# codeslake/RefVSR

Hardware: AMD Instinct MI355X
Metric: 4x SR frames/sec (270p->1080p, RefVSR_small_L1) (higher is better)
Workload: dtype f16

## Files before the change

### refvsr_amd/csrc/common.h

```cpp
#pragma once
#include <stdlib.h>
#include <hip/hip_runtime.h>
#include <hip/hip_fp16.h>
#include <stdint.h>
#include <stdio.h>
#include <string.h>

#include "../../include/refvsr_hip.h"

typedef _Float16 f16;
typedef f16 f16x2 __attribute__((ext_vector_type(2)));
typedef f16 f16x4 __attribute__((ext_vector_type(4)));
typedef f16 f16x8 __attribute__((ext_vector_type(8)));
typedef float f32x4 __attribute__((ext_vector_type(4)));
typedef float f32x16 __attribute__((ext_vector_type(16)));

void refvsr_set_error(const char* fmt, ...);

#define RV_CHECK(cond, ...)                        \
    do {                                           \
        if (!(cond)) {                             \
            refvsr_set_error(__VA_ARGS__);         \
            return 1;                              \
        }                                          \
    } while (0)

#define RV_HIP(call)                                                                  \
    do {                                                                              \
        hipError_t e_ = (call);                                                       \
        if (e_ != hipSuccess) {                                                       \
            refvsr_set_error("%s failed: %s (%s:%d)", #call, hipGetErrorString(e_), __FILE__, __LINE__); \
            return 2;                                                                 \
        }                                                                             \
    } while (0)

#define RV_LAUNCH_CHECK() RV_HIP(hipGetLastError())

static inline int rv_cdiv(int a, int b) { return (a + b - 1) / b; }

#define RV_MAX_DEVICES 16
static inline int rv_device() {
    int d = 0;
    if (hipGetDevice(&d) != hipSuccess || d < 0 || d >= RV_MAX_DEVICES) d = 0;
    return d;
}
static inline int rv_num_cus() {
    static int n_cu[RV_MAX_DEVICES] = {};
    const int d = rv_device();
    if (n_cu[d] == 0) {
        hipDeviceProp_t prop;
        if (hipGetDeviceProperties(&prop, d) == hipSuccess) n_cu[d] = prop.multiProcessorCount;
        if (n_cu[d] <= 0) n_cu[d] = 256;
    }
    return n_cu[d];
}

int rv_stream_cus(hipStream_t st);

__device__ __forceinline__ void rv_tile_range(const int n_tiles, const int g, int& t_begin, int& t_end) {
    const int b = (int)blockIdx.x;
    int rank = b;
    if (g >= 8) {
        const int xcd = b & 7;
        rank = b >> 3;
        for (int y = 0; y < xcd; ++y) rank += (g - y + 7) >> 3;
    }
    const unsigned un = (unsigned)n_tiles, ug = (unsigned)g;
    t_begin = (int)(((unsigned)rank * un) / ug);
    t_end = (int)(((unsigned)(rank + 1) * un) / ug);
}

__device__ __forceinline__ int rv_reflect(int i, int n) {
    i = i < 0 ? -i : i;
    return i >= n ? 2 * (n - 1) - i : i;
}

__device__ __forceinline__ float rv_lrelu(float v, float slope) { return v >= 0.f ? v : v * slope; }

__device__ __forceinline__ float rv_linspace_m1p1(int j, int n) {
    const float step = 2.0f / (float)(n - 1);
    return (j < n / 2) ? (-1.0f + step * (float)j) : (1.0f - step * (float)(n - 1 - j));
}

struct WarpCoord { int x0, y0; float w00, w01, w10, w11; bool v00, v01, v10, v11; };

__device__ __forceinline__ WarpCoord warp_coord_uv(const float u, const float v, int hf, int wf, int hin, int win, int y, int x);
__device__ __forceinline__ WarpCoord warp_coord(const float* flow, int hf, int wf, int hin, int win, int y, int x) {
    const size_t fp = (size_t)y * wf + x;
    return warp_coord_uv(flow[fp], flow[(size_t)hf * wf + fp], hf, wf, hin, win, y, x);
}
__device__ __forceinline__ WarpCoord warp_coord_uv(const float u, const float v, int hf, int wf, int hin, int win, int y, int x) {
    const float gx = rv_linspace_m1p1(x, wf) + u / (((float)win - 1.0f) / 2.0f);
    const float gy = rv_linspace_m1p1(y, hf) + v / (((float)hin - 1.0f) / 2.0f);
    const float xs = ((gx + 1.0f) * (float)win - 1.0f) / 2.0f;
    const float ys = ((gy + 1.0f) * (float)hin - 1.0f) / 2.0f;
    const float fx = floorf(xs), fy = floorf(ys);
    const float tx = xs - fx, ty = ys - fy;
    WarpCoord c;
    c.x0 = (int)fminf(fmaxf(fx, -2.0f), (float)win + 1.0f);
    c.y0 = (int)fminf(fmaxf(fy, -2.0f), (float)hin + 1.0f);
    const bool xin0 = c.x0 >= 0 && c.x0 < win, xin1 = c.x0 + 1 >= 0 && c.x0 + 1 < win;
    const bool yin0 = c.y0 >= 0 && c.y0 < hin, yin1 = c.y0 + 1 >= 0 && c.y0 + 1 < hin;
    c.v00 = xin0 && yin0; c.v01 = xin1 && yin0; c.v10 = xin0 && yin1; c.v11 = xin1 && yin1;
    c.w00 = (1.0f - ty) * (1.0f - tx); c.w01 = (1.0f - ty) * tx;
    c.w10 = ty * (1.0f - tx); c.w11 = ty * tx;
    return c;
}

__device__ __forceinline__ uint4 warp_group16(const unsigned char* x, int pixb, int hin, int win, const WarpCoord& c, int goff) {
    float acc[8] = {0, 0, 0, 0, 0, 0, 0, 0};
    auto tap = [&](bool valid, int yy, int xx, float wgt) {
        if (valid) {
            const f16x8 v = *reinterpret_cast<const f16x8*>(x + ((size_t)yy * win + xx) * pixb + goff);
#pragma unroll
            for (int k = 0; k < 8; ++k) acc[k] += wgt * (float)v[k];
        }
    };
    tap(c.v00, c.y0, c.x0, c.w00);
    tap(c.v01, c.y0, c.x0 + 1, c.w01);
    tap(c.v10, c.y0 + 1, c.x0, c.w10);
    tap(c.v11, c.y0 + 1, c.x0 + 1, c.w11);
    union { f16x8 h; uint4 u; } o;
#pragma unroll
    for (int k = 0; k < 8; ++k) o.h[k] = (f16)acc[k];
    return o.u;
}

__device__ __forceinline__ void rv_bilinear_ac_src(int o, int n_in, int n_out, int& i0, int& i1, float& l1) {
#pragma clang fp contract(off)
    const float sc = n_out > 1 ? (float)(n_in - 1) / (float)(n_out - 1) : 0.0f;
    const float x = (float)o * sc;
    i0 = min((int)x, n_in - 1);
    i1 = min(i0 + 1, n_in - 1);
    l1 = x - (float)i0;
}
__device__ __forceinline__ float rv_bilinear_ac2_at(const float* __restrict__ s, int h, int w, int oy, int ox) {
    int y0, y1, x0, x1;
    float ly, lx;
    rv_bilinear_ac_src(oy, h, 2 * h, y0, y1, ly);
    rv_bilinear_ac_src(ox, w, 2 * w, x0, x1, lx);
    const float wy0 = 1.0f - ly, wx0 = 1.0f - lx;
    const float r0 = fmaf(lx, s[(size_t)y0 * w + x1], fmaf(wx0, s[(size_t)y0 * w + x0], 0.0f));
    const float r1 = fmaf(lx, s[(size_t)y1 * w + x1], fmaf(wx0, s[(size_t)y1 * w + x0], 0.0f));
    return fmaf(ly, r1, fmaf(wy0, r0, 0.0f));
}

__device__ __forceinline__ void rv_cubic_taps(float t, float* wgt) {
    const float A = -0.75f;
    float x = t + 1.0f;
    wgt[0] = ((A * x - 5.0f * A) * x + 8.0f * A) * x - 4.0f * A;
    x = t;
    wgt[1] = ((A + 2.0f) * x - (A + 3.0f)) * x * x + 1.0f;
    x = 1.0f - t;
    wgt[2] = ((A + 2.0f) * x - (A + 3.0f)) * x * x + 1.0f;
    x = 2.0f - t;
    wgt[3] = ((A * x - 5.0f * A) * x + 8.0f * A) * x - 4.0f * A;
}
__device__ __forceinline__ void rv_cubic_src(int o, int n_in, float scale, int* idx, float* wgt) {
    const float x = ((float)o + 0.5f) * scale - 0.5f;
    const float fl = floorf(x);
    const int ix = (int)fl;
    rv_cubic_taps(x - fl, wgt);
#pragma unroll
    for (int k = 0; k < 4; ++k) idx[k] = min(max(ix - 1 + k, 0), n_in - 1);
}
__device__ __forceinline__ float rv_bicubic_at(const float* __restrict__ s, int h, int w, int oy, int ox, float sy, float sx) {
    int iy[4], ix[4];
    float wy[4], wx[4];
    rv_cubic_src(oy, h, sy, iy, wy);
    rv_cubic_src(ox, w, sx, ix, wx);
    float acc = 0.0f;
#pragma unroll
    for (int j = 0; j < 4; ++j) {
        float r = 0.0f;
        const float* row = s + (size_t)iy[j] * w;
#pragma unroll
        for (int i = 0; i < 4; ++i) r = fmaf(wx[i], row[ix[i]], r);
        acc = fmaf(wy[j], r, acc);
    }
    return acc;
}

__device__ __forceinline__ void rv_store_result(void* out, const size_t e, const float v, const int fmt) {
    if (fmt == REFVSR_RESULT_F32) reinterpret_cast<float*>(out)[e] = v;
    else if (fmt == REFVSR_RESULT_F16) reinterpret_cast<f16*>(out)[e] = (f16)v;
    else reinterpret_cast<unsigned char*>(out)[e] = (unsigned char)__float2int_rn(v * 255.0f);
}

__host__ __device__ inline int rv_keven(int ks, int ncg) {
    const int ce = (ncg + 1) >> 1, co = ncg >> 1;
    return ks * (((ks + 1) >> 1) * ce + (ks >> 1) * co);
}
__host__ __device__ inline int rv_ksteps(int ks, int ncg) { return (ks * ks * ncg + (rv_keven(ks, ncg) & 1) + 3) / 4; }
__host__ __device__ inline int rv_kslot(int ty, int tx, int cg, int ks, int ncg) {
    const int ce = (ncg + 1) >> 1, co = ncg >> 1;
    const int p = (tx + cg) & 1;
    const int c0 = p ? co : ce, c1 = p ? ce : co;
    const int row = ((ks + 1) >> 1) * c0 + (ks >> 1) * c1;
    const int rank = ty * row + ((tx + 1) >> 1) * c0 + (tx >> 1) * c1 + (cg >> 1);
    if (!p) return rank;
    const int E = rv_keven(ks, ncg);
    return E + (E & 1) + rank;
}
__host__ __device__ inline int rv_kpad_slot(int j, int ks, int ncg) {
    const int E = rv_keven(ks, ncg);
    return ((E & 1) && j == 0) ? E : ks * ks * ncg + j;
}
__device__ __forceinline__ int rv_pix16(int n) { return (n < 4 || n >= 12) ? ((n & 7) << 1) : (((n - 4) << 1) | 1); }
```

### refvsr_amd/csrc/conv_mfma.hip

```cpp
#include <type_traits>

#include "common.h"
#include <stdlib.h>

#define CONV_CH 8
#define CONV_RES_MAX 16
#define CONV_XPF 8
#define CONV_TW 32

struct ConvArgs {
    const unsigned char* src0; const unsigned char* src1;
    int c0, c1, ncg0, ncg, ps;
    int pixb0, pixb1;
    int h_in, w_in, h_out, w_out;
    int ks, stride, pad;
    int LH, LW;
    int G, S;
    float inv_ncg;
    const uint4* wpack; const float* bias;
    int cout;
    float act_slope, post_slope;
    const unsigned char* mul; int mul_c;
    const unsigned char* res; int res_c;
    int out_mode; void* out; int out_c;
// ... 455 lines not shown
            auto ld128 = [](const unsigned addr) {
                u32x4 v;
                asm volatile("ds_read_b128 %0, %1" : "=v"(v) : "v"(addr));
                return make_uint4(v[0], v[1], v[2], v[3]);
            };
            auto tie = [](uint4& r) {
                u32x4 t = {r.x, r.y, r.z, r.w};
                asm volatile("" : "+v"(t));
                r = make_uint4(t[0], t[1], t[2], t[3]);
            };
            auto wait_set = [&](uint4 (&a)[NA], uint4 (&b)[TILES]) {
                asm volatile("s_waitcnt lgkmcnt(%0)" :: "n"(NA + TILES) : "memory");
#pragma unroll
                for (int i = 0; i < NA; ++i) tie(a[i]);
#pragma unroll
                for (int t = 0; t < TILES; ++t) tie(b[t]);
            };
            static_assert(NA + TILES <= 15, "lgkmcnt range");
            auto compute_chunk = [&](const unsigned wslot, const int s0, const int ns) {
                unsigned toff[CONV_CH];
#pragma unroll
                for (int j = 0; j < CONV_CH; ++j)
                    asm volatile("ds_read_b32 %0, %1" : "=v"(toff[j]) : "v"(lds_tab + (unsigned)(((s0 + min(j, ns - 1)) * 4 + q) * 4)));
                asm volatile("s_waitcnt lgkmcnt(0)" ::: "memory");
#pragma unroll
                for (int j = 0; j < CONV_CH; ++j) asm volatile("" : "+v"(toff[j]));
                const unsigned wa = wslot + (unsigned)lane * 16;
                auto load_set = [&](auto jc, uint4 (&a)[NA], uint4 (&b)[TILES]) {
                    constexpr int j = decltype(jc)::value;
                    const unsigned wj = wa + (unsigned)min(j, ns - 1) * (NA * 1024);
#pragma unroll
                    for (int i = 0; i < NA; ++i) {
                        u32x4 v;
                        asm volatile("ds_read_b128 %0, %1 offset:%2" : "=v"(v) : "v"(wj), "n"(i * 1024));
                        a[i] = make_uint4(v[0], v[1], v[2], v[3]);
                    }
#pragma unroll
                    for (int t = 0; t < TILES; ++t) b[t] = ld128(pbaddr[t] + toff[j]);
                };
                uint4 a0[NA], b0[TILES], a1[NA], b1[TILES];
                load_set(std::integral_constant<int, 0>{}, a0, b0);
#define RV_RING_PAIR(J)                                                                     \
                load_set(std::integral_constant<int, (J) + 1>{}, a1, b1);                   \
                wait_set(a0, b0);                                                           \
                __builtin_amdgcn_sched_barrier(0);                                          \
                if ((J) < ns) mfma_step(a0, b0);                                            \
                load_set(std::integral_constant<int, (J) + 2>{}, a0, b0);                   \
                wait_set(a1, b1);                                                           \
                __builtin_amdgcn_sched_barrier(0);                                          \
                if ((J) + 1 < ns) mfma_step(a1, b1);
                RV_RING_PAIR(0) RV_RING_PAIR(2) RV_RING_PAIR(4)
#undef RV_RING_PAIR
                static_assert(CONV_CH == 8, "the ring loop is unrolled for 8 K-steps per chunk");
                load_set(std::integral_constant<int, 7>{}, a1, b1);
                wait_set(a0, b0);
                __builtin_amdgcn_sched_barrier(0);
                if (6 < ns) mfma_step(a0, b0);
                asm volatile("s_waitcnt lgkmcnt(0)" ::: "memory");
#pragma unroll
                for (int i = 0; i < NA; ++i) tie(a1[i]);
#pragma unroll
                for (int t = 0; t < TILES; ++t) tie(b1[t]);
                __builtin_amdgcn_sched_barrier(0);
                if (7 < ns) mfma_step(a1, b1);
            };
            const int n_chunks = (p.S + CONV_CH - 1) / CONV_CH;
            zero_acc();
            int slot_r = 0;
            for (int c = 0; c < n_chunks; ++c) {
                const int after = min(NS - 2, n_chunks - 1 - c);
                if (after <= 0) asm volatile("s_waitcnt vmcnt(0)" ::: "memory");
                else if (after == 1) asm volatile("s_waitcnt vmcnt(%0)" :: "n"(PPW) : "memory");
                else asm volatile("s_waitcnt vmcnt(%0)" :: "n"(2 * PPW) : "memory");
                asm volatile("s_waitcnt lgkmcnt(0)" ::: "memory");
                __builtin_amdgcn_s_barrier();
                asm volatile("" ::: "memory");
                if (c + NS - 1 < n_chunks) { issue(c + NS - 1, slot_w); slot_w = slot_w + 1 == NS ? 0 : slot_w + 1; }
                compute_chunk(lds_wl + (unsigned)slot_r * SLOT, c * CONV_CH, min(CONV_CH, p.S - c * CONV_CH));
                slot_r = slot_r + 1 == NS ? 0 : slot_r + 1;
            }
        } else {
            constexpr int WPT = (CONV_CH * MT * WFR * 64) / NT;
            const int n_chunks = (p.S + CONV_CH - 1) / CONV_CH;
            static_assert(WPT <= 12, "prefetch register set");
            uint4 w0, w1, w2, w3, w4, w5, w6, w7, w8, w9, w10, w11;
    #define RV_W_ALL(OP) OP(0) OP(1) OP(2) OP(3) OP(4) OP(5) OP(6) OP(7) OP(8) OP(9) OP(10) OP(11)
    #define RV_W_LOAD(k) if constexpr (WPT > k) w##k = g[min(tid + k * NT, n16n - 1)];
    #define RV_W_STORE(k) if constexpr (WPT > k) { if (tid + k * NT < n16n) d[tid + k * NT] = w##k; }
            {
                const int n16 = min(CONV_CH, p.S) * MT * WFR * 64;
                uint4* d = reinterpret_cast<uint4*>(wl);
                for (int i = tid; i < n16; i += NT) d[i] = wsrc[i];
            }
            zero_acc();
            __syncthreads();
            for (int c = 0; c < n_chunks; ++c) {
                const int s0 = c * CONV_CH;
                const int ns = min(CONV_CH, p.S - s0);
                const bool has_next = (c + 1 < n_chunks);
                const int sn = has_next ? s0 + CONV_CH : s0;
                const int n16n = min(CONV_CH, p.S - sn) * MT * WFR * 64;
                {
                    const uint4* g = wsrc + (size_t)sn * MT * WFR * 64;
                    RV_W_ALL(RV_W_LOAD)
                }
                compute_steps(wl, s0, ns);
                if (has_next) {
                    __syncthreads();
                    uint4* d = reinterpret_cast<uint4*>(wl);
                    RV_W_ALL(RV_W_STORE)
                    __syncthreads();
                }
            }
        }
        epilogue(ty0, tx0, tid);
    }
}

static int g_wg_cap = 0;
extern "C" int refvsr_set_conv_workgroup_cap(int cap) {
    g_wg_cap = cap > 0 ? cap : 0;
    return 0;
}

extern "C" int refvsr_kslot(int ty, int tx, int cg, int ksize, int ncg) { return rv_kslot(ty, tx, cg, ksize, ncg); }
extern "C" int refvsr_ksteps(int ksize, int ncg) { return rv_ksteps(ksize, ncg); }

template <int MT, int TILES, bool F32, bool GATHER, bool RESIDENT, int EPI = 0, int NW = 4, bool HI1 = false>
static int launch_conv(ConvArgs& a, int nz, size_t lds, hipStream_t st) {
    static bool attr_done[RV_MAX_DEVICES] = {};
    const int dev = rv_device();
    if (!attr_done[dev]) {
        RV_HIP(hipFuncSetAttribute(reinterpret_cast<const void*>(&conv_mfma_kernel<MT, TILES, F32, GATHER, RESIDENT, EPI, NW, HI1>),
                                   hipFuncAttributeMaxDynamicSharedMemorySize, 160 * 1024));
        attr_done[dev] = true;
    }
    int gx = a.n_xy;
    if (RESIDENT) {
        static size_t occ_lds[RV_MAX_DEVICES][4] = {};
        static int occ_val[RV_MAX_DEVICES][4] = {};
        static int slot[RV_MAX_DEVICES] = {};
        int occ = 0;
        for (int i = 0; i < 4; ++i)
            if (occ_lds[dev][i] == lds && occ_val[dev][i] > 0) occ = occ_val[dev][i];
        if (occ == 0) {
            RV_HIP(hipOccupancyMaxActiveBlocksPerMultiprocessor(&occ, conv_mfma_kernel<MT, TILES, F32, GATHER, RESIDENT, EPI, NW, HI1>, NW * 64, lds));
            if (occ < 1) occ = 1;
            occ_lds[dev][slot[dev] & 3] = lds; occ_val[dev][slot[dev] & 3] = occ; ++slot[dev];
        }
        int cap = (rv_stream_cus(st) * occ / (nz * (a.batch > 1 ? a.batch : 1))) & ~7;
        if (cap < 8) cap = 8;
        if (g_wg_cap > 0) cap = g_wg_cap;
        if (gx > cap) gx = cap;
    }
    a.grid = gx;
    hipLaunchKernelGGL((conv_mfma_kernel<MT, TILES, F32, GATHER, RESIDENT, EPI, NW, HI1>), dim3(gx, a.batch > 1 ? a.batch : 1, nz), dim3(NW * 64), lds, st, a);
    RV_LAUNCH_CHECK();
    return 0;
}

extern "C" int refvsr_conv_mfma(const RefvsrConv* d, void* stream) {
    RV_CHECK(d != nullptr, "conv: null descriptor");
    const bool f32 = d->f32 == 1;
    const bool hi1 = d->f32 == 2;
    RV_CHECK(d->f32 >= 0 && d->f32 <= 2, "conv: weight mode (f32) must be 0, 1 or 2");
    const int cgrp = f32 ? 4 : 8;
    const int esz = f32 ? 4 : 2;
    RV_CHECK(d->src0 && d->c0 > 0 && d->c0 % cgrp == 0, "conv: src0/c0 invalid (c0=%d)", d->c0);
    RV_CHECK((d->src1 == nullptr) == (d->c1 == 0) && d->c1 % cgrp == 0, "conv: src1/c1 invalid (c1=%d)", d->c1);
    RV_CHECK(d->ksize >= 1 && d->ksize <= 7 && d->stride >= 1 && d->pad >= 0, "conv: bad geometry");
    RV_CHECK(d->h_in > 0 && d->w_in > 0 && d->h_out > 0 && d->w_out > 0, "conv: bad sizes");
    RV_CHECK(d->wpack && d->bias && d->out, "conv: null weights/bias/out");
    RV_CHECK(d->mt_per_block >= 1 && d->mt_per_block <= 3, "conv: mt_per_block must be 1..3");
    RV_CHECK(d->cout >= 1, "conv: cout");
    if (d->out_mode != REFVSR_OUT_PLANAR32) {
        RV_CHECK(d->cout % 4 == 0 && d->out_c % 4 == 0, "conv: nhwc16 output needs cout %% 4 == 0");
        RV_CHECK(d->res_planar == nullptr, "conv: res_planar only with planar output");
    }
    if (d->out_mode == REFVSR_OUT_NHWC16_SHUFFLE2)
        RV_CHECK(d->cout % 16 == 0 && !d->mul && !d->res && !f32 && d->out_c >= d->cout / 4 && d->out_c - d->cout / 4 <= 4,
                 "conv: pixel-shuffle output constraints");
    RV_CHECK(refvsr_init() == 0, "init failed");

    ConvArgs a;
    memset(&a, 0, sizeof(a));
    a.src0 = (const unsigned char*)d->src0; a.src1 = (const unsigned char*)d->src1;
    a.c0 = d->c0; a.c1 = d->c1;
    a.pixb0 = d->c0 * esz; a.pixb1 = d->c1 * esz;
    a.ncg0 = d->c0 / cgrp; a.ncg = (d->c0 + d->c1) / cgrp;
    a.ps = a.ncg | 1;
    a.h_in = d->h_in; a.w_in = d->w_in; a.h_out = d->h_out; a.w_out = d->w_out;
    a.ks = d->ksize; a.stride = d->stride; a.pad = d->pad;
    a.G = d->ksize * d->ksize * a.ncg;
    a.S = rv_ksteps(d->ksize, a.ncg);
    RV_CHECK(a.S == d->ksteps, "conv: ksteps mismatch (descriptor %d, geometry %d)", d->ksteps, a.S);
    a.inv_ncg = 1.0f / (float)a.ncg;
    a.wpack = (const uint4*)d->wpack; a.bias = d->bias; a.cout = d->cout;
    a.act_slope = d->act_slope; a.post_slope = d->post_slope;
    a.mul = (const unsigned char*)d->mul; a.mul_c = d->mul_c;
    a.res = (const unsigned char*)d->res; a.res_c = d->res_c;
    a.out_mode = d->out_mode; a.out = d->out; a.out_c = d->out_c;
    a.res_planar = d->res_planar; a.add_const = d->add_const;
    a.clamp_lo = d->clamp_lo; a.clamp_hi = d->clamp_hi;
    RV_CHECK(d->batch >= 0 && d->batch <= 65535, "conv: batch out of range (%d)", d->batch);
    a.batch = d->batch > 1 ? d->batch : 1;
    if (a.batch > 1) {
        RV_CHECK(!d->mul && !d->res, "conv: batch > 1 takes no mul / res operands");
        RV_CHECK(d->bs_src0 % 16 == 0 && d->bs_src1 % 16 == 0 && d->bs_out % 8 == 0 && d->bs_res_planar % 4 == 0, "conv: batch strides must keep the maps aligned");
        RV_CHECK(d->bs_src0 > 0 && d->bs_out > 0 && (!d->src1 || d->bs_src1 > 0) && (!d->res_planar || d->bs_res_planar > 0), "conv: batch strides missing");
        a.bs_src0 = d->bs_src0; a.bs_src1 = d->bs_src1; a.bs_out = d->bs_out; a.bs_res_planar = d->bs_res_planar;
    }

    const int MT = d->mt_per_block;
    const int n_mt = (d->cout + 15) / 16;
    const int nz = (n_mt + MT - 1) / MT;
    a.tab_bytes = ((a.S * 4 * 4 + 15) / 16) * 16;
    const int wfr_kb = MT * ((f32 || hi1) ? 1 : 2) * 1024;
    static const bool no_resident = getenv("REFVSR_CONV_NO_PERSIST") != nullptr;
    const size_t LDS_MAX = 160 * 1024;

    int tiles = 4;
    size_t lds = 0;
    auto tile_bytes = [&](int tl) {
        a.LH = (tl * 2 - 1) * a.stride + a.ks;
        a.LW = (CONV_TW - 1) * a.stride + a.ks;
        return (size_t)a.LH * a.LW * a.ps * 16;
    };
    bool resident = false, one_wg = false;
    bool w16 = false;
    static const int res_max = getenv("REFVSR_CONV_RES_MAX") ? atoi(getenv("REFVSR_CONV_RES_MAX")) : CONV_RES_MAX;
    if (!no_resident && !hi1 && a.S <= res_max && a.S <= CONV_RES_MAX) {
        int best_wg = 0;
        static const int force_tiles = getenv("REFVSR_CONV_TILES") ? atoi(getenv("REFVSR_CONV_TILES")) : 0;
        for (int tl = 4; tl >= 2; tl -= 2) {
            if (force_tiles && tl != force_tiles) continue;
            const size_t tb = tile_bytes(tl);
            const size_t need = (size_t)a.tab_bytes + (size_t)a.S * wfr_kb + tb;
            const int chunks = a.LH * a.LW * a.ncg;
            const int wg = need <= LDS_MAX ? (int)(LDS_MAX / need) : 0;
            if (chunks > CONV_XPF * 256 || wg == 0) continue;
            if (a.LH > 31 || a.LW > 127 || a.ncg > 127) continue;
            if (best_wg == 0 || (best_wg < 2 && wg > best_wg)) { best_wg = wg; tiles = tl; lds = need; resident = true; }
        }
        if (resident) { a.wl_bytes = a.S * wfr_kb; tile_bytes(tiles); one_wg = best_wg == 1; }
        static const bool no_w16 = getenv("REFVSR_CONV_NO_W16") != nullptr;
        if (resident && one_wg && tiles == 4 && !f32 && !no_w16 && (MT == 2 || MT == 3)) {
            const size_t tb = tile_bytes(8);
            const size_t need = (size_t)a.tab_bytes + (size_t)a.S * wfr_kb + tb;
            const int chunks = a.LH * a.LW * a.ncg;
            if (need <= LDS_MAX && chunks <= 4096 && a.LH <= 31 && a.LW <= 127) { tiles = 8; lds = need; w16 = true; }
            else tile_bytes(tiles);
        }
    }
    if (!resident) {
        const size_t slot = (size_t)CONV_CH * wfr_kb;
        const int n_chunks = (a.S + CONV_CH - 1) / CONV_CH;
        auto ring_for = [&](int tl, size_t budget) {
            const size_t fixed = (size_t)a.tab_bytes + tile_bytes(tl);
            if (fixed + 2 * slot > budget) return 0;
            int ns = (int)((budget - fixed) / slot);
            if (ns > 4) ns = 4;
            if (ns > n_chunks + 1) ns = n_chunks + 1 > 2 ? n_chunks + 1 : 2;
            return ns;
        };
        static const int force_ring = getenv("REFVSR_CONV_RING") ? atoi(getenv("REFVSR_CONV_RING")) : 0;
        const bool big = (long long)d->h_out * d->w_out > 64 * 1024;
        int ns = 0;
        tiles = 4;
        if (big) ns = ring_for(4, LDS_MAX / 2);
        if (!ns && big) { tiles = 2; ns = ring_for(2, LDS_MAX / 2); }
        if (!ns) { tiles = 4; ns = ring_for(4, LDS_MAX); }
        if (!ns) { tiles = 2; ns = ring_for(2, LDS_MAX); }
        if (ns) {
            if (force_ring >= 2 && force_ring < ns) ns = force_ring;
            a.ring = ns;
            a.wl_bytes = (int)(ns * slot);
            lds = (size_t)a.tab_bytes + (size_t)a.wl_bytes + tile_bytes(tiles);
        } else {
            a.gather = 1;
            a.ring = 1;
            tiles = 4;
            a.LH = a.LW = 0;
            a.wl_bytes = (int)slot;
            lds = (size_t)a.tab_bytes + (size_t)a.wl_bytes;
            RV_CHECK(d->h_in < 60000 && d->w_in < 60000, "conv: frame too large for gather-mode coordinates");
        }
        one_wg = !a.gather && lds > LDS_MAX / 2;
    }
    static const bool no_nw8 = getenv("REFVSR_CONV_NO_NW8") != nullptr;
    const int n_tiles8 = rv_cdiv(d->w_out, CONV_TW) * rv_cdiv(d->h_out, 8);
    const bool nw8 = tiles == 4 && !f32 && !a.gather && !no_nw8 && (one_wg || n_tiles8 <= 2048);
    static const bool no_prefetch = getenv("REFVSR_CONV_NO_PREFETCH") != nullptr;
    a.prefetch = no_prefetch ? 0 : 1;
    a.tiles_x = rv_cdiv(d->w_out, CONV_TW);
    a.n_xy = a.tiles_x * rv_cdiv(d->h_out, tiles * 2);
    hipStream_t st = (hipStream_t)stream;
    if (a.gather) {
        RV_CHECK(!f32 && !hi1, "conv: gather mode is built for the fp16 hi+lo path only");
        if (MT == 1) return launch_conv<1, 4, false, true, false>(a, nz, lds, st);
        if (MT == 2) return launch_conv<2, 4, false, true, false>(a, nz, lds, st);
        return launch_conv<3, 4, false, true, false>(a, nz, lds, st);
    }
    if (hi1) {
        RV_CHECK(!a.gather && MT <= 2, "conv: single-fp16 weights are built for the streamed stride-1 convs (MT=%d)", MT);
        const bool nw8h = tiles == 4 && !no_nw8 && (one_wg || n_tiles8 <= 2048);
        if (nw8h) return MT == 1 ? launch_conv<1, 2, false, false, false, 0, 8, true>(a, nz, lds, st)
                                 : launch_conv<2, 2, false, false, false, 0, 8, true>(a, nz, lds, st);
        if (tiles == 4) return MT == 1 ? launch_conv<1, 4, false, false, false, 0, 4, true>(a, nz, lds, st)
                                       : launch_conv<2, 4, false, false, false, 0, 4, true>(a, nz, lds, st);
        return MT == 1 ? launch_conv<1, 2, false, false, false, 0, 4, true>(a, nz, lds, st)
                       : launch_conv<2, 2, false, false, false, 0, 4, true>(a, nz, lds, st);
    }
    static const bool no_lean = getenv("REFVSR_CONV_NO_LEAN_EPI") != nullptr;
    const bool lean = resident && !f32 && !no_lean && d->out_mode == REFVSR_OUT_NHWC16 && d->act_slope >= 0.f && d->act_slope <= 1.f &&
                      d->post_slope >= 0.f && d->post_slope <= 1.f &&
                      (long long)d->h_out * d->w_out * (long long)(d->out_c > d->mul_c ? (d->out_c > d->res_c ? d->out_c : d->res_c)
                                                                                       : (d->mul_c > d->res_c ? d->mul_c : d->res_c)) < (1ll << 31);
#define RV_CONV_CASE(M, T)                                                                                \
    if (MT == M && tiles == T) {                                                                          \
        if (f32) return resident ? launch_conv<M, T, true, false, true>(a, nz, lds, st)                   \
                                 : launch_conv<M, T, true, false, false>(a, nz, lds, st);                 \
        if (lean) return launch_conv<M, T, false, false, true, 1>(a, nz, lds, st);                        \
        return resident ? launch_conv<M, T, false, false, true>(a, nz, lds, st)                           \
                        : launch_conv<M, T, false, false, false>(a, nz, lds, st);                         \
    }
    if (w16) {
        if (MT == 3) return lean ? launch_conv<3, 2, false, false, true, 1, 16>(a, nz, lds, st) : launch_conv<3, 2, false, false, true, 0, 16>(a, nz, lds, st);
        return lean ? launch_conv<2, 2, false, false, true, 1, 16>(a, nz, lds, st) : launch_conv<2, 2, false, false, true, 0, 16>(a, nz, lds, st);
    }
    if (nw8) {
#define RV_CONV_CASE8(M)                                                                                  \
        if (MT == M) {                                                                                    \
            if (lean) return launch_conv<M, 2, false, false, true, 1, 8>(a, nz, lds, st);                 \
            return resident ? launch_conv<M, 2, false, false, true, 0, 8>(a, nz, lds, st)                 \
                            : launch_conv<M, 2, false, false, false, 0, 8>(a, nz, lds, st);               \
        }
        RV_CONV_CASE8(1) RV_CONV_CASE8(2) RV_CONV_CASE8(3)
#undef RV_CONV_CASE8
    }
    if (!no_nw8 && f32 && tiles == 2 && !a.gather && (MT == 1 || MT == 2)) {
        if (MT == 1) return resident ? launch_conv<1, 1, true, false, true, 0, 8>(a, nz, lds, st) : launch_conv<1, 1, true, false, false, 0, 8>(a, nz, lds, st);
        return resident ? launch_conv<2, 1, true, false, true, 0, 8>(a, nz, lds, st) : launch_conv<2, 1, true, false, false, 0, 8>(a, nz, lds, st);
    }
    RV_CONV_CASE(1, 2) RV_CONV_CASE(1, 4)
    RV_CONV_CASE(2, 2) RV_CONV_CASE(2, 4)
    RV_CONV_CASE(3, 2) RV_CONV_CASE(3, 4)
#undef RV_CONV_CASE
    refvsr_set_error("conv: no kernel for MT=%d tiles=%d", MT, tiles);
    return 1;
}
```

Before: 235.3.

## Add specialized 7x7 SPyNet conv kernel with pipelined weight streaming

Adds a dedicated MFMA kernel for the stride-1 7x7 SPyNet convolutions (32->64, 64->32, 32->16 channels) and routes the single-fp16-weight conv path to it when shapes match. The kernel stages an input tile in LDS and streams weight chunks into a multi-slot LDS ring via global_load_lds. It uses hand-scheduled ds_read and waitcnt double-buffering around the MFMAs. This targets the heavy 7x7 flow-network convolutions that the generic conv kernel handles less efficiently, at the cost of fixed shape-specific configurations and inline-asm fragility.

```diff
diff --git a/refvsr_amd/csrc/common.h b/refvsr_amd/csrc/common.h
--- a/refvsr_amd/csrc/common.h
+++ b/refvsr_amd/csrc/common.h
@@ -56,6 +56,8 @@
 }
 
 int rv_stream_cus(hipStream_t st);
+
+int rv_spynet7_conv(const RefvsrConv* d, hipStream_t st);
 
 __device__ __forceinline__ void rv_tile_range(const int n_tiles, const int g, int& t_begin, int& t_end) {
     const int b = (int)blockIdx.x;
diff --git a/refvsr_amd/csrc/conv_mfma.hip b/refvsr_amd/csrc/conv_mfma.hip
--- a/refvsr_amd/csrc/conv_mfma.hip
+++ b/refvsr_amd/csrc/conv_mfma.hip
@@ -781,6 +781,8 @@
         return launch_conv<3, 4, false, true, false>(a, nz, lds, st);
     }
     if (hi1) {
+        const int r7 = rv_spynet7_conv(d, st);
+        if (r7 >= 0) return r7;
         RV_CHECK(!a.gather && MT <= 2, "conv: single-fp16 weights are built for the streamed stride-1 convs (MT=%d)", MT);
         const bool nw8h = tiles == 4 && !no_nw8 && (one_wg || n_tiles8 <= 2048);
         if (nw8h) return MT == 1 ? launch_conv<1, 2, false, false, false, 0, 8, true>(a, nz, lds, st)
diff --git a/refvsr_amd/csrc/spynet7.hip b/refvsr_amd/csrc/spynet7.hip
--- /dev/null
+++ b/refvsr_amd/csrc/spynet7.hip
@@ -0,0 +1,291 @@
+#include <type_traits>
+#include <utility>
+
+#include "common.h"
+
+#define SP7_TW 32
+
+struct Spynet7Args {
+    const unsigned char* src;
+    const unsigned char* wpack;
+    const float* bias;
+    unsigned char* out;
+    int h, w;
+    int tiles_x;
+    int pk;
+    float act_slope, post_slope;
+    unsigned long long bs_src, bs_out;
+};
+
+template <class F, int... J>
+__device__ __forceinline__ void sp7_unroll(F& f, std::integer_sequence<int, J...>) { (f(std::integral_constant<int, J>{}), ...); }
+
+template <int CIN, int MT, int NW, int TR, int CH, int NS>
+struct Sp7Cfg {
+    static constexpr int NCG = CIN / 8;
+    static constexpr int PS = NCG | 1;
+    static constexpr int KS = 7;
+    static constexpr int S = (KS * KS * NCG + 3) / 4;
+    static constexpr int G = KS * KS * NCG;
+    static constexpr int LH = TR + KS - 1, LW = SP7_TW + KS - 1;
+    static constexpr int NT = NW * 64;
+    static constexpr int P = 2 * TR / NW;
+    static constexpr int TAB = ((S * 4 * 4 + 15) / 16) * 16;
+    static constexpr int SLOT = CH * MT * 1024;
+    static constexpr int TILE = LH * LW * PS * 16;
+    static constexpr int LDS = TAB + NS * SLOT + TILE;
+    static constexpr int NCHUNK = (S + CH - 1) / CH;
+    static constexpr int PPW = CH * MT / NW;
+    static_assert(CIN % 8 == 0 && (NCG & (NCG - 1)) == 0, "channel groups");
+    static_assert(G == 4 * S, "the SPyNet shapes need no zero K-blocks");
+    static_assert(P >= 1 && (P % 2 == 0 || P == 1) && NW * P == 2 * TR, "pixel groups per wave");
+    static_assert(PPW >= 1 && PPW * NW == CH * MT, "pieces per wave and chunk");
+    static_assert(MT + P <= 15, "lgkmcnt range");
+    static_assert(LDS <= 160 * 1024, "LDS");
+};
+
+template <int CIN, int MT, int NW, int TR, int CH, int NS, int WPE>
+__global__ __launch_bounds__(NW * 64) __attribute__((amdgpu_waves_per_eu(WPE, WPE))) void spynet7_kernel(Spynet7Args p) {
+    using C = Sp7Cfg<CIN, MT, NW, TR, CH, NS>;
+    constexpr int NCG = C::NCG, PS = C::PS, KS = C::KS, S = C::S, LW = C::LW, LH = C::LH, NT = C::NT, P = C::P;
+    extern __shared__ __attribute__((aligned(16))) unsigned char smem[];
+    int* tab = reinterpret_cast<int*>(smem);
+    unsigned char* wl = smem + C::TAB;
+    unsigned char* tile = wl + NS * C::SLOT;
+
+    asm volatile("" :: "s"(p.src), "s"(p.wpack), "s"(p.bias), "s"(p.out), "s"(p.h), "s"(p.w), "s"(p.tiles_x), "s"(p.pk));
+    {
+        const unsigned long long bi = blockIdx.y;
+        p.src += bi * p.bs_src;
+        p.out += bi * p.bs_out;
+    }
+    const int tid = threadIdx.x;
+    const int lane = tid & 63;
+    const int wave = tid >> 6;
+    const int q = lane >> 4;
+    const int lp = rv_pix16(lane & 15);
+    const int tl = blockIdx.x;
+    const int tyi = tl / p.tiles_x;
+    const int tx0 = (tl - tyi * p.tiles_x) * SP7_TW;
+    const int ty0 = tyi * TR;
+
+    for (int g = tid; g < C::G; g += NT) {
+        const int tap = g / NCG, cg = g % NCG;
+        const int ty = tap / KS, tx = tap % KS;
+        tab[rv_kslot(ty, tx, cg, KS, NCG)] = ((ty * LW + tx) * PS + cg) * 16;
+    }
+
+    const int wv = __builtin_amdgcn_readfirstlane(wave);
+    const int pk = p.pk;
+    const unsigned char* gw = p.wpack + lane * 16;
+    auto issue = [&](const int c, const int slot) {
+        unsigned char* l = wl + slot * C::SLOT;
+#pragma unroll
+        for (int j = 0; j < C::PPW; ++j) {
+            const int pc = wv + j * NW;
+            const int s = min(c * CH + pc / MT, S - 1);
+            const int m = pc % MT;
+            const int zg = m / pk, mm = m - zg * pk;
+            const unsigned char* g = gw + ((size_t)(zg * S + s) * pk + mm) * 1024;
+            __builtin_amdgcn_global_load_lds((const __attribute__((address_space(1))) void*)g,
+                                             (__attribute__((address_space(3))) void*)(l + pc * 1024), 16, 0, 0);
+        }
+    };
+    int slot_w = 0;
+#pragma unroll
+    for (int c = 0; c < NS - 1 && c < C::NCHUNK; ++c) { issue(c, slot_w); slot_w = slot_w + 1 == NS ? 0 : slot_w + 1; }
+
+    {
+        const int iy0 = ty0 - 3, ix0 = tx0 - 3;
+        constexpr int total = LH * LW * NCG;
+        constexpr int SB = 8;
+        for (int idx0 = tid; idx0 < total; idx0 += SB * NT) {
+            uint4 sv[SB];
+            int sd[SB];
+#pragma unroll
+            for (int k = 0; k < SB; ++k) {
+                const int idx = min(idx0 + k * NT, total - 1);
+                const int r = idx / (LW * NCG);
+                const int i = idx - r * (LW * NCG);
+                const int c = i / NCG, cg = i % NCG;
+                const int iy = iy0 + r, ix = ix0 + c;
+                const bool ok = (unsigned)iy < (unsigned)p.h && (unsigned)ix < (unsigned)p.w;
+                const size_t pix = (size_t)min(max(iy, 0), p.h - 1) * p.w + min(max(ix, 0), p.w - 1);
+                uint4 v = *reinterpret_cast<const uint4*>(p.src + pix * (CIN * 2) + cg * 16);
+                const unsigned keep = ok ? 0xffffffffu : 0u;
+                v.x &= keep; v.y &= keep; v.z &= keep; v.w &= keep;
+                sv[k] = v;
+                sd[k] = ((r * LW + c) * PS + cg) * 16;
+            }
+#pragma unroll
+            for (int k = 0; k < SB; ++k)
+                if (idx0 + k * NT < total) *reinterpret_cast<uint4*>(tile + sd[k]) = sv[k];
+        }
+    }
+
+    float4 bias_r[MT];
+#pragma unroll
+    for (int m = 0; m < MT; ++m) bias_r[m] = *reinterpret_cast<const float4*>(p.bias + m * 16 + q * 4);
+
+    typedef unsigned u32x4 __attribute__((ext_vector_type(4)));
+    const unsigned lds_tab = (unsigned)(size_t)(__attribute__((address_space(3))) unsigned char*)reinterpret_cast<unsigned char*>(tab);
+    const unsigned lds_wl = (unsigned)(size_t)(__attribute__((address_space(3))) unsigned char*)wl;
+    const unsigned lds_tile = (unsigned)(size_t)(__attribute__((address_space(3))) unsigned char*)tile;
+    const int g0 = wave * P;
+    const unsigned pb = lds_tile + (unsigned)((((g0 >> 1) * LW + (g0 & 1) * 16 + lp) * PS) * 16);
+    auto goff = [](const int t) { return ((t >> 1) * LW + (t & 1) * 16) * PS * 16; };
+    static_assert(P == 1 || (((P >> 1) - 1) * LW + 16) * PS * 16 < 65536, "ds_read immediate offset range");
+
+    f32x4 acc[MT][P];
+#pragma unroll
+    for (int m = 0; m < MT; ++m)
+#pragma unroll
+        for (int t = 0; t < P; ++t) acc[m][t] = (f32x4){0.f, 0.f, 0.f, 0.f};
+
+    auto tie = [](uint4& r) {
+        u32x4 t = {r.x, r.y, r.z, r.w};
+        asm volatile("" : "+v"(t));
+        r = make_uint4(t[0], t[1], t[2], t[3]);
+    };
+    auto mfma_step = [&](const uint4 (&a)[MT], const uint4 (&b)[P]) {
+#pragma unroll
+        for (int t = 0; t < P; ++t) {
+            const f16x8 bv = *reinterpret_cast<const f16x8*>(&b[t]);
+#pragma unroll
+            for (int m = 0; m < MT; ++m)
+                acc[m][t] = __builtin_amdgcn_mfma_f32_16x16x32_f16(*reinterpret_cast<const f16x8*>(&a[m]), bv, acc[m][t], 0, 0, 0);
+        }
+    };
+    auto compute_chunk = [&](const unsigned wslot, const int s0, const int ns) {
+        unsigned toff[CH];
+#pragma unroll
+        for (int j = 0; j < CH; ++j)
+            asm volatile("ds_read_b32 %0, %1" : "=v"(toff[j]) : "v"(lds_tab + (unsigned)(((s0 + min(j, ns - 1)) * 4 + q) * 4)));
+        asm volatile("s_waitcnt lgkmcnt(0)" ::: "memory");
+#pragma unroll
+        for (int j = 0; j < CH; ++j) asm volatile("" : "+v"(toff[j]));
+        const unsigned wa = wslot + (unsigned)lane * 16;
+        auto load_set = [&](auto jc, uint4 (&a)[MT], uint4 (&b)[P]) {
+            constexpr int j = decltype(jc)::value;
+            const unsigned wj = wa + (unsigned)min(j, ns - 1) * (MT * 1024);
+#pragma unroll
+            for (int m = 0; m < MT; ++m) {
+                u32x4 v;
+                asm volatile("ds_read_b128 %0, %1 offset:%2" : "=v"(v) : "v"(wj), "n"(m * 1024));
+                a[m] = make_uint4(v[0], v[1], v[2], v[3]);
+            }
+            const unsigned bj = pb + toff[j];
+#pragma unroll
+            for (int t = 0; t < P; ++t) {
+                u32x4 v;
+                asm volatile("ds_read_b128 %0, %1 offset:%2" : "=v"(v) : "v"(bj), "n"(P == 1 ? 0 : goff(t)));
+                b[t] = make_uint4(v[0], v[1], v[2], v[3]);
+            }
+        };
+        uint4 a0[MT], b0[P], a1[MT], b1[P];
+        auto step = [&](auto jc) {
+            constexpr int j = decltype(jc)::value;
+            uint4 (&ac)[MT] = (j & 1) ? a1 : a0;
+            uint4 (&bc)[P] = (j & 1) ? b1 : b0;
+            uint4 (&an)[MT] = (j & 1) ? a0 : a1;
+            uint4 (&bn)[P] = (j & 1) ? b0 : b1;
+            if constexpr (j + 1 < CH) {
+                load_set(std::integral_constant<int, j + 1>{}, an, bn);
+                asm volatile("s_waitcnt lgkmcnt(%0)" :: "n"(MT + P) : "memory");
+            } else {
+                asm volatile("s_waitcnt lgkmcnt(0)" ::: "memory");
+            }
+#pragma unroll
+            for (int m = 0; m < MT; ++m) tie(ac[m]);
+#pragma unroll
+            for (int t = 0; t < P; ++t) tie(bc[t]);
+            __builtin_amdgcn_sched_barrier(0);
+            if (j < ns) mfma_step(ac, bc);
+        };
+        load_set(std::integral_constant<int, 0>{}, a0, b0);
+        sp7_unroll(step, std::make_integer_sequence<int, CH>{});
+    };
+
+    int slot_r = 0;
+    for (int c = 0; c < C::NCHUNK; ++c) {
+        const int after = min(NS - 2, C::NCHUNK - 1 - c);
+        if (after <= 0) asm volatile("s_waitcnt vmcnt(0)" ::: "memory");
+        else if (after == 1) asm volatile("s_waitcnt vmcnt(%0)" :: "n"(C::PPW) : "memory");
+        else asm volatile("s_waitcnt vmcnt(%0)" :: "n"(2 * C::PPW) : "memory");
+        asm volatile("s_waitcnt lgkmcnt(0)" ::: "memory");
+        __builtin_amdgcn_s_barrier();
+        asm volatile("" ::: "memory");
+        if (c + NS - 1 < C::NCHUNK) { issue(c + NS - 1, slot_w); slot_w = slot_w + 1 == NS ? 0 : slot_w + 1; }
+        compute_chunk(lds_wl + (unsigned)slot_r * C::SLOT, c * CH, min(CH, S - c * CH));
+        slot_r = slot_r + 1 == NS ? 0 : slot_r + 1;
+    }
+
+    f16* outp = reinterpret_cast<f16*>(p.out);
+#pragma unroll
+    for (int t = 0; t < P; ++t) {
+        const int gi = g0 + t;
+        const int oy = ty0 + (gi >> 1);
+        const int ox = tx0 + (gi & 1) * 16 + lp;
+        if (oy >= p.h || ox >= p.w) continue;
+        const size_t opix = (size_t)oy * p.w + ox;
+#pragma unroll
+        for (int m = 0; m < MT; ++m) {
+            const int co0 = m * 16 + q * 4;
+            float y[4];
+            const float4 bv = bias_r[m];
+            y[0] = acc[m][t][0] + bv.x; y[1] = acc[m][t][1] + bv.y;
+            y[2] = acc[m][t][2] + bv.z; y[3] = acc[m][t][3] + bv.w;
+#pragma unroll
+            for (int i = 0; i < 4; ++i) y[i] = rv_lrelu(y[i], p.act_slope);
+            if (p.post_slope != 1.0f) {
+#pragma unroll
+                for (int i = 0; i < 4; ++i) y[i] = rv_lrelu(y[i], p.post_slope);
+            }
+            const f16x4 o = {(f16)y[0], (f16)y[1], (f16)y[2], (f16)y[3]};
+            *reinterpret_cast<f16x4*>(outp + opix * (MT * 16) + co0) = o;
+        }
+    }
+}
+
+template <int CIN, int MT, int NW, int TR, int CH, int NS, int WPE>
+static int launch_spynet7(const RefvsrConv* d, hipStream_t st) {
+    using C = Sp7Cfg<CIN, MT, NW, TR, CH, NS>;
+    static bool attr_done[RV_MAX_DEVICES] = {};
+    const int dev = rv_device();
+    if (!attr_done[dev]) {
+        RV_HIP(hipFuncSetAttribute(reinterpret_cast<const void*>(&spynet7_kernel<CIN, MT, NW, TR, CH, NS, WPE>),
+                                   hipFuncAttributeMaxDynamicSharedMemorySize, C::LDS));
+        attr_done[dev] = true;
+    }
+    Spynet7Args a;
+    memset(&a, 0, sizeof(a));
+    a.src = (const unsigned char*)d->src0;
+    a.wpack = (const unsigned char*)d->wpack;
+    a.bias = d->bias;
+    a.out = (unsigned char*)d->out;
+    a.h = d->h_out; a.w = d->w_out;
+    a.tiles_x = rv_cdiv(d->w_out, SP7_TW);
+    a.pk = d->mt_per_block;
+    a.act_slope = d->act_slope; a.post_slope = d->post_slope;
+    const int batch = d->batch > 1 ? d->batch : 1;
+    if (batch > 1) { a.bs_src = d->bs_src0; a.bs_out = d->bs_out; }
+    const int n_xy = a.tiles_x * rv_cdiv(d->h_out, TR);
+    hipLaunchKernelGGL((spynet7_kernel<CIN, MT, NW, TR, CH, NS, WPE>), dim3(n_xy, batch, 1), dim3(NW * 64), C::LDS, st, a);
+    RV_LAUNCH_CHECK();
+    return 0;
+}
+
+int rv_spynet7_conv(const RefvsrConv* d, hipStream_t st) {
+    static const int off = getenv("REFVSR_SPYNET7_OFF") != nullptr;
+    if (off) return -1;
+    if (d->f32 != 2 || d->ksize != 7 || d->stride != 1 || d->pad != 3 || d->src1 != nullptr || d->c1 != 0) return -1;
+    if (d->out_mode != REFVSR_OUT_NHWC16 || d->mul || d->res || d->res_planar) return -1;
+    if (d->h_in != d->h_out || d->w_in != d->w_out || d->out_c != d->cout) return -1;
+    const int mt = d->mt_per_block;
+    if (mt < 1 || mt > 2) return -1;
+    if (d->batch > 1 && (d->bs_src0 % 16 != 0 || d->bs_out % 8 != 0)) return -1;
+    if (d->c0 == 32 && d->cout == 64 && mt == 2) return launch_spynet7<32, 4, 4, 8, 4, 2, 2>(d, st);
+    if (d->c0 == 64 && d->cout == 32 && mt == 2) return launch_spynet7<64, 2, 8, 16, 8, 2, 2>(d, st);
+    if (d->c0 == 32 && d->cout == 16 && mt == 1) return launch_spynet7<32, 1, 4, 8, 8, 2, 2>(d, st);
+    return -1;
+}
```

Result: faster. 238.1 (median of 6 runs) (+1.2%).
